# qfall/tools

Measured on AMD Instinct MI355X. Metric: preimages/sec (whole node) + HBM-BW% for samp_p, n=512 q~2^30 batch=4096, higher is better.
Workload: dtype f64+int64

## Files before the change

### tools_amd/csrc/psf_np_kernels.hpp

```cpp
#pragma once
#include <type_traits>
#include "psf_kernels.hpp"

namespace psf {

constexpr int NP_NB = 64;

__host__ __device__ inline size_t np_panel_rowblocks(size_t J) { return (J * NP_NB + 127) / 128; }
__host__ __device__ inline size_t np_panel_base(size_t J) { return 4 * ((J * J) / 4); }

__global__ __launch_bounds__(256) void k_np_gram(const int32_t* __restrict__ St, const double* __restrict__ Gt, size_t d, double* __restrict__ Gd) {
  __shared__ double sB[16][65];
  __shared__ double sG[16][65];
  const size_t j0 = (size_t)blockIdx.y * 64, i0 = (size_t)blockIdx.x * 64;
  const int tid = threadIdx.x, tx = tid & 15, ty = tid >> 4;
  if (i0 > j0 + 63) {
    for (int e = tid; e < 64 * 64; e += 256) {
      const size_t j = j0 + (e >> 6), i = i0 + (e & 63);
      if (j < d && i < d) Gd[j * d + i] = 0.0;
    }
    return;
  }
  double acc[4][4];
#pragma unroll
  for (int a = 0; a < 4; ++a)
#pragma unroll
    for (int b = 0; b < 4; ++b) acc[a][b] = 0.0;
  for (size_t t0 = 0; t0 < d; t0 += 16) {
    for (int e = tid; e < 64 * 16; e += 256) {
      const int r = e >> 4, tt = e & 15;
      const size_t t = t0 + tt;
      sB[tt][r] = (j0 + r < d && t < d) ? (double)St[(j0 + r) * d + t] : 0.0;
      sG[tt][r] = (i0 + r < d && t < d) ? Gt[(i0 + r) * d + t] : 0.0;
    }
    __syncthreads();
#pragma unroll
    for (int tt = 0; tt < 16; ++tt) {
      double bv[4], gv[4];
#pragma unroll
      for (int a = 0; a < 4; ++a) { bv[a] = sB[tt][ty * 4 + a]; gv[a] = sG[tt][tx * 4 + a]; }
#pragma unroll
      for (int a = 0; a < 4; ++a)
#pragma unroll
        for (int b = 0; b < 4; ++b) acc[a][b] = fma(bv[a], gv[b], acc[a][b]);
    }
    __syncthreads();
  }
#pragma unroll
  for (int a = 0; a < 4; ++a)
#pragma unroll
    for (int b = 0; b < 4; ++b) {
      const size_t j = j0 + ty * 4 + a, i = i0 + tx * 4 + b;
      if (j < d && i < d) Gd[j * d + i] = j > i ? acc[a][b] : 0.0;
    }
}

__global__ void k_np_pack_panels(const double* __restrict__ Gd, size_t d, size_t nblk, double* __restrict__ Gp) {
  const size_t total = np_panel_base(nblk) * TR_CHUNK;
  for (size_t g = (size_t)blockIdx.x * blockDim.x + threadIdx.x; g < total; g += (size_t)gridDim.x * blockDim.x) {
    const size_t chunk = g / TR_CHUNK;
    const int pos = (int)(g % TR_CHUNK);
    size_t J = (size_t)(2.0 * sqrt((double)(chunk / 4)));
    while (np_panel_base(J + 1) <= chunk) ++J;
    while (np_panel_base(J) > chunk) --J;
    const size_t rel = chunk - np_panel_base(J), rb = rel / 4, kc = rel % 4;
    const int ks = pos >> 9, tile = (pos >> 6) & 7, ln = pos & 63;
    const size_t i = rb * 128 + tile * 16 + (ln & 15);
    const size_t j = J * NP_NB + kc * 16 + ks * 4 + (ln >> 4);
    Gp[g] = (i < J * NP_NB && j < d) ? Gd[j * d + i] : 0.0;
  }
}
constexpr int NP_TRI = 2048;
__global__ void k_np_pack_inblock(const double* __restrict__ Gd, size_t d, size_t nblk, double* __restrict__ Gin) {
  const size_t total = nblk * NP_TRI;
  for (size_t g = (size_t)blockIdx.x * blockDim.x + threadIdx.x; g < total; g += (size_t)gridDim.x * blockDim.x) {
    const size_t J = g / NP_TRI, e = g % NP_TRI;
    double v = 0.0;
    if (e < (size_t)NP_NB * (NP_NB - 1) / 2) {
      size_t l = (size_t)((1.0 + sqrt(1.0 + 8.0 * (double)e)) * 0.5);
      while (l * (l - 1) / 2 > e) --l;
      while ((l + 1) * l / 2 <= e) ++l;
      const size_t li = e - l * (l - 1) / 2;
      const size_t j = J * NP_NB + l, i = J * NP_NB + li;
      if (j < d) v = Gd[j * d + i];
    }
// ... 740 lines not shown
  const int wr = wave >> 1, wc = wave & 1;
  const size_t row0 = (size_t)bi * TR_BM + wr * 32, col0 = (size_t)bj * TR_BN + wc * 64;
  d4 acc[2][4];
#pragma unroll
  for (int i = 0; i < 2; ++i)
#pragma unroll
    for (int j = 0; j < 4; ++j)
#pragma unroll
      for (int r = 0; r < 4; ++r) acc[i][j][r] = T[(row0 + i * 16 + (lane >> 4) + 4 * r) * ldt + col0 + j * 16 + (lane & 15)];
  const int nk = 4 * job.nsub;
  auto stage_load = [&](int kc, int buf) {
    const size_t Jb = (size_t)(job.J_first - (kc >> 2));
    const double* ga = Gp + (np_panel_base(Jb) + (size_t)bi * 4 + (size_t)(kc & 3)) * TR_CHUNK + lane * 2;
    const double* gb = Zf + ((size_t)bj * nkb + Jb * (NP_NB / 16) + (size_t)(kc & 3)) * TR_CHUNK + lane * 2;
    double* la = smem + buf * (2 * TR_CHUNK);
#pragma unroll
    for (int i = 0; i < 2; ++i) {
      const int piece = wave * 2 + i;
      __builtin_amdgcn_global_load_lds(ga + piece * 128, (lds_void_ptr)(la + piece * 128), 16, 0, 0);
      __builtin_amdgcn_global_load_lds(gb + piece * 128, (lds_void_ptr)(la + TR_CHUNK + piece * 128), 16, 0, COH ? 16 : 0);
    }
  };
  stage_load(0, 0);
  asm volatile("s_waitcnt vmcnt(0)" ::: "memory");
  __syncthreads();
  for (int kc = 0; kc < nk; ++kc) {
    const int cur = kc & 1;
    if (kc + 1 < nk) stage_load(kc + 1, cur ^ 1);
    const double* sA = smem + cur * (2 * TR_CHUNK);
    const double* sB = sA + TR_CHUNK;
#pragma unroll
    for (int ks = 0; ks < TR_BK / 4; ++ks) {
      double av[2], bv[4];
#pragma unroll
      for (int i = 0; i < 2; ++i) av[i] = -sA[(ks * 8 + wr * 2 + i) * 64 + lane];
#pragma unroll
      for (int i = 0; i < 4; ++i) bv[i] = sB[(ks * 8 + wc * 4 + i) * 64 + lane];
#pragma unroll
      for (int i = 0; i < 2; ++i)
#pragma unroll
        for (int j = 0; j < 4; ++j) acc[i][j] = __builtin_amdgcn_mfma_f64_16x16x4f64(av[i], bv[j], acc[i][j], 0, 0, 0);
    }
    asm volatile("s_waitcnt vmcnt(0)" ::: "memory");
    __syncthreads();
  }
#pragma unroll
  for (int i = 0; i < 2; ++i)
#pragma unroll
    for (int j = 0; j < 4; ++j)
#pragma unroll
      for (int r = 0; r < 4; ++r) {
        const size_t row = row0 + i * 16 + (lane >> 4) + 4 * r;
        if (row >= job.row_lo && row < job.row_hi) {
          if (COH) __hip_atomic_store(T + row * ldt + col0 + j * 16 + (lane & 15), acc[i][j][r], __ATOMIC_RELAXED, __HIP_MEMORY_SCOPE_AGENT);
          else T[row * ldt + col0 + j * 16 + (lane & 15)] = acc[i][j][r];
        }
      }
}

struct NpStepJobs { NpUpdateJob job[3]; unsigned ntiles[3]; };

template <int G>
__global__ __launch_bounds__(512, 4) void k_np_step(NpSampleArgs a, size_t dim, size_t J, uint64_t seed, uint32_t tag, uint64_t first_index, size_t B, unsigned nS,
                                                    NpStepJobs jobs, int nbj, const double* __restrict__ Gp, double* __restrict__ Tm) {
  extern __shared__ __attribute__((aligned(16))) unsigned char np_smem[];
  unsigned id = blockIdx.x;
  if (id < nS) { np_sample_body<G>(np_smem, id, a, dim, J, seed, tag, first_index, B); return; }
  id -= nS;
#pragma unroll
  for (int q = 0; q < 3; ++q) {
    if (id < jobs.ntiles[q]) { np_update_tile(reinterpret_cast<double*>(np_smem), id, jobs.job[q], nbj, Gp, a.Zf, a.nkb, Tm, a.ldt); return; }
    id -= jobs.ntiles[q];
  }
}

constexpr int NP_GW = 64;
constexpr int NP_WALK_SLOTS = 3;
struct NpWalkSync {
  unsigned* zcount;
  unsigned* tready;
  unsigned* abort;
  unsigned nblk_stride;
  unsigned spin_limit;
};

__device__ __forceinline__ bool np_walk_wait(const unsigned* word, unsigned target, unsigned* abort_word, unsigned spin_limit, int* s_flag) {
  if (threadIdx.x == 0) {
    int ok = 1;
    unsigned spins = 0;
    while (__hip_atomic_load(word, __ATOMIC_RELAXED, __HIP_MEMORY_SCOPE_AGENT) < target) {
      __builtin_amdgcn_s_sleep(2);
      if ((++spins & 255u) == 0 && __hip_atomic_load(abort_word, __ATOMIC_RELAXED, __HIP_MEMORY_SCOPE_AGENT) != 0) { ok = 0; break; }
      if (spins >= spin_limit) { __hip_atomic_store(abort_word, 1u, __ATOMIC_RELAXED, __HIP_MEMORY_SCOPE_AGENT); ok = 0; break; }
    }
    *s_flag = ok;
  }
  __syncthreads();
  const int ok = *s_flag;
  __syncthreads();
  return ok != 0;
}

template <int G>
__device__ __forceinline__ void np_walk_sampler(unsigned char* smem, unsigned wg, const NpSampleArgs& a, size_t dim, size_t nblk, uint64_t seed, uint32_t tag,
                                                uint64_t first_index, size_t B, const NpWalkSync& sy) {
  int* s_flag = reinterpret_cast<int*>(smem + 65536 - 16);
  const unsigned grp = wg / (unsigned)(NP_GW / (4 * G));
  long long zr[G];
#pragma unroll
  for (int s = 0; s < G; ++s) zr[s] = 0;
  for (size_t J = nblk; J-- > 0;) {
    if (J + 2 < nblk) {
      if (!np_walk_wait(sy.tready + (size_t)grp * sy.nblk_stride + J, 1u, sy.abort, sy.spin_limit, s_flag)) return;
    }
    np_sample_body<G, true, true>(smem, wg, a, dim, J, seed, tag, first_index, B, zr);
    asm volatile("s_waitcnt vmcnt(0)" ::: "memory");
    __syncthreads();
    if (threadIdx.x == 0 && J >= 2) __hip_atomic_fetch_add(sy.zcount + (size_t)grp * sy.nblk_stride + J, 1u, __ATOMIC_RELAXED, __HIP_MEMORY_SCOPE_AGENT);
  }
}

__device__ __forceinline__ void np_walk_updater(unsigned char* smem, unsigned grp, unsigned ul, unsigned ug, unsigned need, const NpSampleArgs& a, size_t nblk,
                                                const double* __restrict__ Gp, double* __restrict__ T, const NpWalkSync& sy) {
  double* s_z = reinterpret_cast<double*>(smem);
  int* s_flag = reinterpret_cast<int*>(smem + 65536 - 16);
  int* s_arr = reinterpret_cast<int*>(smem + 65536 - 32);
  const int tid = threadIdx.x, lane = tid & 63;
  const int wave = __builtin_amdgcn_readfirstlane(tid >> 6);
  const size_t col0 = (size_t)grp * NP_GW;
  const size_t ldt = a.ldt;
  const uint32_t t_lane = (uint32_t)(((size_t)(lane >> 4) * ldt + (size_t)(lane & 15)) * sizeof(double));
  const uint32_t f_lane = (uint32_t)(lane * sizeof(double));
  auto t_at = [&](size_t row, size_t col) -> double* {
    return reinterpret_cast<double*>(reinterpret_cast<char*>(T + row * ldt + col) + t_lane);
  };
  d4 acc[NP_WALK_SLOTS][4];
  long blk[NP_WALK_SLOTS];
#pragma unroll
  for (int sl = 0; sl < NP_WALK_SLOTS; ++sl) {
    const long k = 2 * sl + (wave >> 2);
    const long Jb = (long)ul + k * (long)ug;
    blk[sl] = Jb + 2 < (long)nblk ? Jb : -1;
    const size_t row0 = (size_t)(blk[sl] < 0 ? 0 : blk[sl]) * NP_NB + (size_t)(wave & 3) * 16;
#pragma unroll
    for (int nf = 0; nf < 4; ++nf)
#pragma unroll
      for (int r = 0; r < 4; ++r) acc[sl][nf][r] = blk[sl] < 0 ? 0.0 : *t_at(row0 + 4 * r, col0 + nf * 16);
  }
  if (tid == 0) *s_arr = 0;
  const size_t bj = col0 / TR_BN;
  const int t0 = (int)((col0 % TR_BN) / 16);
  for (size_t J = nblk; J-- > 2;) {
    if (!np_walk_wait(sy.zcount + (size_t)grp * sy.nblk_stride + J, need, sy.abort, sy.spin_limit, s_flag)) return;
    {
      const double* zsrc = a.Zf + (bj * a.nkb + J * (NP_NB / 16)) * TR_CHUNK;
#pragma unroll
      for (int i = 0; i < 8; ++i) {
        const int e = i * 8 + wave;
        const int kstep = e >> 2, nf = e & 3, kc = kstep >> 2, ks = kstep & 3;
        const double* src = reinterpret_cast<const double*>(reinterpret_cast<const char*>(zsrc + (size_t)kc * TR_CHUNK + (size_t)((ks * 8 + t0 + nf) * 64)) + f_lane);
        s_z[e * 64 + lane] = __hip_atomic_load(src, __ATOMIC_RELAXED, __HIP_MEMORY_SCOPE_AGENT);
      }
    }
    __syncthreads();
    const long Ju = (long)J - 2;
#pragma unroll
    for (int pass = 0; pass < 2; ++pass) {
#pragma unroll
      for (int sl = 0; sl < NP_WALK_SLOTS; ++sl) {
        const bool urgent = blk[sl] == Ju;
        if (blk[sl] < 0 || blk[sl] > Ju || urgent != (pass == 0)) continue;
        const size_t i0 = (size_t)blk[sl] * NP_NB + (size_t)(wave & 3) * 16;
        const double* ga = Gp + (np_panel_base(J) + (i0 / 128) * 4) * TR_CHUNK + ((i0 % 128) / 16) * 64;
#pragma unroll
        for (int kstep = 0; kstep < 16; ++kstep) {
          const double av = -*reinterpret_cast<const double*>(reinterpret_cast<const char*>(ga + (size_t)(kstep >> 2) * TR_CHUNK + (kstep & 3) * 512) + f_lane);
#pragma unroll
          for (int nf = 0; nf < 4; ++nf) acc[sl][nf] = __builtin_amdgcn_mfma_f64_16x16x4f64(av, s_z[(kstep * 4 + nf) * 64 + lane], acc[sl][nf], 0, 0, 0);
        }
        if (urgent) {
#pragma unroll
          for (int nf = 0; nf < 4; ++nf)
#pragma unroll
            for (int r = 0; r < 4; ++r)
              __hip_atomic_store(t_at((size_t)Ju * NP_NB + (size_t)(wave & 3) * 16 + 4 * r, col0 + nf * 16), acc[sl][nf][r], __ATOMIC_RELAXED, __HIP_MEMORY_SCOPE_AGENT);
          asm volatile("s_waitcnt vmcnt(0)" ::: "memory");
          if (lane == 0) {
            const int prev = __hip_atomic_fetch_add(s_arr, 1, __ATOMIC_RELAXED, __HIP_MEMORY_SCOPE_WORKGROUP);
            if ((prev & 3) == 3) __hip_atomic_store(sy.tready + (size_t)grp * sy.nblk_stride + (size_t)Ju, 1u, __ATOMIC_RELAXED, __HIP_MEMORY_SCOPE_AGENT);
          }
        }
      }
    }
    __syncthreads();
  }
}

template <int G>
__global__ __launch_bounds__(512, 4) void k_np_walk(NpSampleArgs a, size_t dim, size_t nblk, uint64_t seed, uint32_t tag, uint64_t first_index, size_t B, unsigned nS,
                                                    unsigned ngroups, unsigned ug, const double* __restrict__ Gp, double* __restrict__ Tm, NpWalkSync sy) {
  extern __shared__ __attribute__((aligned(16))) unsigned char np_smem[];
  unsigned id = blockIdx.x;
  if (id < nS) {
    np_walk_sampler<G>(np_smem, id, a, dim, nblk, seed, tag, first_index, B, sy);
  } else {
    id -= nS;
    const unsigned grp = id / ug, ul = id % ug;
    if (grp >= ngroups) return;
    const unsigned per = (unsigned)(NP_GW / (4 * G));
    const unsigned first = grp * per, need = nS - first < per ? nS - first : per;
    np_walk_updater(np_smem, grp, ul, ug, need, a, nblk, Gp, Tm, sy);
  }
}

template <int G>
__global__ __launch_bounds__(512, 4) void k_np_walk_solo(NpSampleArgs a, size_t dim, size_t nblk, uint64_t seed, uint32_t tag, uint64_t first_index, size_t B, const double* __restrict__ Gp,
                                                         double* __restrict__ Tm, const unsigned* __restrict__ only_if, unsigned long long* __restrict__ reruns) {
  extern __shared__ __attribute__((aligned(16))) unsigned char np_smem[];
  if (__hip_atomic_load(only_if, __ATOMIC_RELAXED, __HIP_MEMORY_SCOPE_AGENT) == 0) return;
  const unsigned wg = blockIdx.x;
  const int tid = threadIdx.x, lane = tid & 63;
  const int wave = __builtin_amdgcn_readfirstlane(tid >> 6);
  if (wg == 0 && tid == 0) atomicAdd(reruns, 1ull);
  long long zr[G];
#pragma unroll
  for (int s = 0; s < G; ++s) zr[s] = 0;
  const size_t b = (size_t)wg * 4 * G + (size_t)wave;
  const bool owner = wave < 4 * G && b < B;
  for (size_t J = nblk; J-- > 0;) {
    if (J + 2 < nblk) {
      __builtin_amdgcn_fence(__ATOMIC_ACQUIRE, "agent");
      if (owner) {
        const size_t i = J * NP_NB + (size_t)lane;
        double t = Tm[i * a.ldt + b];
        const double* zb = a.Zf + (b / TR_BN) * a.nkb * TR_CHUNK;
        const int bc = (int)(b % TR_BN);
        for (size_t Jb = nblk; Jb-- > J + 2;) {
          const double* gp = Gp + (np_panel_base(Jb) + (i / 128) * 4) * TR_CHUNK;
          const double* zp = zb + Jb * (NP_NB / 16) * TR_CHUNK;
#pragma unroll 4
          for (int kc = 0; kc < NP_NB / 16; ++kc)
#pragma unroll
            for (int kk = 0; kk < 16; ++kk)
              t = fma(-zp[(size_t)kc * TR_CHUNK + tr_chunk_pos(bc, kk)], gp[(size_t)kc * TR_CHUNK + tr_chunk_pos((int)(i % 128), kk)], t);
        }
        __hip_atomic_store(Tm + i * a.ldt + b, t, __ATOMIC_RELAXED, __HIP_MEMORY_SCOPE_AGENT);
      }
      asm volatile("s_waitcnt vmcnt(0)" ::: "memory");
      __syncthreads();
    }
    np_sample_body<G, true, true>(np_smem, wg, a, dim, J, seed, tag, first_index, B, zr);
    asm volatile("s_waitcnt vmcnt(0)" ::: "memory");
    __syncthreads();
  }
}

#ifdef PSF_EXPERIMENTS
template <int G>
struct NpWalk2Jobs {
  const double* Gp; double* T; const double* Zf;
  const unsigned* zcount_g; unsigned* tready_g; unsigned* abort_w; int* s_arr;
  size_t ldt, nkb, col0, bj;
  unsigned need, spin_limit;
  int nblk, t0, hw, HW, lane;
  uint32_t t_lane, f_lane;
  int Jn, fi, zmin;
  bool aborted;

  __device__ __forceinline__ bool spin(const unsigned* word, unsigned target) {
    unsigned spins = 0;
    while (__hip_atomic_load(word, __ATOMIC_RELAXED, __HIP_MEMORY_SCOPE_AGENT) < target) {
      if (aborted) return false;
      __builtin_amdgcn_s_sleep(2);
      if ((++spins & 255u) == 0 && __hip_atomic_load(abort_w, __ATOMIC_RELAXED, __HIP_MEMORY_SCOPE_AGENT) != 0) { aborted = true; return false; }
      if (spins >= spin_limit) { __hip_atomic_store(abort_w, 1u, __ATOMIC_RELAXED, __HIP_MEMORY_SCOPE_AGENT); aborted = true; return false; }
    }
    return true;
  }
  __device__ __forceinline__ bool wait_word(const unsigned* w) { return spin(w, 1u); }
  __device__ __forceinline__ int imax(int J) const {
    const int fmax = 4 * (J - 2) + 3;
    return fmax >= hw ? (fmax - hw) / HW : -1;
  }
  __device__ __forceinline__ double* t_at(size_t row, size_t col) const {
    return reinterpret_cast<double*>(reinterpret_cast<char*>(T + row * ldt + col) + t_lane);
// ... 356 lines not shown
```

### tools_amd/csrc/psfgpv_impl.hpp

```cpp

#include <algorithm>
#include "psf_hip_util.hpp"
struct NpBatch {
  size_t bcap = 0;
  DevArr<double> dTm;
  DevArr<double> dZf;
  DevArr<int8_t> dZ8;
  DevArr<double> dC0p;
  DevArr<uint64_t> dSol;
  DevArr<double> dC1;
  DevArr<int64_t> dE1;
  DevArr<unsigned> dWalk;
  DevArr<unsigned char> dZocc;
};
struct NpLane : NpBatch {
  size_t ld = 0, zplane = 0, walk_words = 0;
  DevArr<int> dFlags;
  int* dFail = nullptr;
};

struct psfgpv_handle {
  psfp_handle* base = nullptr;
  double s = 0;
  size_t n = 0, m = 0, dim = 0;
  DevArr<int32_t> dSt;
  DevArr<double> dGt;
  DevArr<double> dNorm2;
  DevArr<SampleZParams> dSz;
  DevArr<uint64_t> dT;
  DevArr<uint32_t> dPiv;
  size_t nblk = 0, dpad = 0, nrb = 0, nkc = 0, nkb = 0;
  DevArr<double> dGp;
  DevArr<double> dGin;
  DevArr<double> dGnx;
  DevArr<NpRow> dRows;
  DevArr<double> dBpiv;
  DevArr<int8_t> dB8;
  bool basis_hi = false, basis_generic = false;
  DevArr<unsigned char> dBocc;
  int np_combine = 1;
  NpLane ln[2];
  int last_lanes = 1;
  bool two_pass = false;
  size_t nkd = 0;
  DevArr<double> dBfull;
  int np_walk = -1;
  int cus = 0;
  int walk_slots[3] = {0, 0, 0};
  unsigned walk_spins = 1u << 22;
  int last_form = 0, last_G = 0;
  int last_parts = 1;
  int split_delay_us = 0;
  int np_split = 0;
  Stream sh[2];
  Event evFork, evHalf[2];
  int np_g = 0;
  int np_immediate = -1;
  bool has_key = false;
  bool timing = false;
  bool last_generic = false;
  Event ev[3];
  hipStream_t last_stream = nullptr;
};

static psf_status gpv_finish_basis(psfgpv_handle* g, bool compute_gso) {
  const size_t d = g->dim;
  KeygenClock kc("psfgpv");
  if (compute_gso) {
    hipLaunchKernelGGL(k_i32_to_f64, dim3(grid_for(d * d)), dim3(256), 0, 0, g->dSt, g->dGt, d * d);
    DevBuf dinfo;
    HIP_TRY(dinfo.alloc(sizeof(int)));
    HIP_TRY(dinfo.zero(sizeof(int)));
    if (gso_blocked(nullptr, g->dGt, d, d, dinfo.as<int>()) != hipSuccess) return PSF_ERR_HIP;
    int info = 0;
    dinfo.download(&info, sizeof(int));
    if (info != 0) return PSF_ERR_PARAM;
    kc.mark("  gso_blocked");
  }
  hipLaunchKernelGGL(k_row_norm2_chain, dim3((unsigned)((d + 63) / 64)), dim3(64), 0, 0, g->dGt, d, g->dNorm2);
  HIP_TRY(hipGetLastError());
  std::vector<double> norm2(d);
  HIP_TRY(hipMemcpy(norm2.data(), g->dNorm2, d * sizeof(double), hipMemcpyDeviceToHost));
  std::vector<SampleZParams> sz(d);
  for (size_t i = 0; i < d; ++i) {
    if (!(norm2[i] > 0.0)) return PSF_ERR_PARAM;
    sz[i] = make_sample_z_params(g->s / std::sqrt(norm2[i]));
  }
  HIP_TRY(hipMemcpy(g->dSz, sz.data(), d * sizeof(SampleZParams), hipMemcpyHostToDevice));
  {
    std::vector<NpRow> rows(g->nblk * NP_NB, NpRow{0.0, 0.f, 0, 1, 0, 0, 16});
    for (size_t i = 0; i < d; ++i) {
      const SampleZParams& p = sz[i];
      const bool fast = p.n_int < (1u << 24) && p.c6 < (1ll << 24);
      rows[i] = NpRow{1.0 / norm2[i], (float)(p.inv_s * 2.1289340388624525), fast ? (int32_t)p.c6 : 0, p.n_int, p.thr_int, p.thr_frac, fast ? p.sh : 0u};
    }
    HIP_TRY(hipMemcpy(g->dRows, rows.data(), rows.size() * sizeof(NpRow), hipMemcpyHostToDevice));
  }
  kc.mark("  norms, SampleZ rows");
  {
    DevBuf gram;
    HIP_TRY(gram.alloc(d * d * sizeof(double)));
    double* dGd = gram.as<double>();
    const unsigned tiles = (unsigned)((d + 63) / 64);
    hipLaunchKernelGGL(k_np_gram, dim3(tiles, tiles), dim3(256), 0, 0, g->dSt, g->dGt, d, dGd);
    if (np_panel_base(g->nblk))
      hipLaunchKernelGGL(k_np_pack_panels, dim3(grid_for(np_panel_base(g->nblk) * TR_CHUNK, 256, 256 * 64)), dim3(256), 0, 0, dGd, d, g->nblk, g->dGp);
    hipLaunchKernelGGL(k_np_pack_inblock, dim3(grid_for(g->nblk * NP_TRI)), dim3(256), 0, 0, dGd, d, g->nblk, g->dGin);
    hipLaunchKernelGGL(k_np_pack_next, dim3(grid_for(g->nblk * NP_NB * NP_NB)), dim3(256), 0, 0, dGd, d, g->nblk, g->dGnx);
    HIP_TRY(hipGetLastError());
    HIP_TRY(hipDeviceSynchronize());
  }
  kc.mark("  gram + packing");
  {
    DevBuf dinfo;
    HIP_TRY(dinfo.alloc(2 * sizeof(int)));
    HIP_TRY(dinfo.zero(2 * sizeof(int)));
    hipLaunchKernelGGL(k_np_pack_basis8, dim3(grid_for(g->dpad * g->dpad, 256, 256 * 64)), dim3(256), 0, 0, g->dSt, d, g->dpad, g->dB8, dinfo.as<int>());
    int info[2] = {0, 0};
    HIP_TRY(dinfo.download(info, sizeof(info)));
    g->basis_generic = info[0] != 0;
    g->basis_hi = info[1] != 0;
    hipLaunchKernelGGL(k_np_occ_basis, dim3((unsigned)(g->nrb * g->nrb), 2), dim3(256), 0, 0, g->dB8, g->dpad, (int)g->nrb, g->dBocc);
    HIP_TRY(hipGetLastError());
  }
  return PSF_OK;
}

static psf_status gpv_build_solver(psfgpv_handle* g) {
  psfp_handle* b = g->base;
  std::vector<uint64_t> A(b->n * b->m);
  HIP_TRY(hipMemcpy(A.data(), b->dA, A.size() * sizeof(uint64_t), hipMemcpyDeviceToHost));
  std::vector<uint32_t> piv;
  std::vector<uint64_t> T;
  const psf_status rc = solve_precompute(A.data(), b->n, b->m, b->q, piv, T);
  if (rc != PSF_OK) return rc;
  {
    const size_t nn = b->n;
    std::vector<size_t> order(nn);
    for (size_t r = 0; r < nn; ++r) order[r] = r;
    std::sort(order.begin(), order.end(), [&](size_t x, size_t y) { return piv[x] < piv[y]; });
    std::vector<uint32_t> piv2(nn);
    std::vector<uint64_t> T2(T.size());
    for (size_t r = 0; r < nn; ++r) {
      piv2[r] = piv[order[r]];
      for (size_t t = 0; t < nn; ++t) T2[r * nn + t] = T[order[r] * nn + t];
    }
    piv.swap(piv2);
    T.swap(T2);
  }
  {
    const size_t nn = b->n;
    std::vector<uint64_t> Tt(T.size());
    for (size_t r = 0; r < nn; ++r)
      for (size_t t = 0; t < nn; ++t) Tt[t * nn + r] = T[r * nn + t];
    HIP_TRY(hipMemcpy(g->dT, Tt.data(), Tt.size() * sizeof(uint64_t), hipMemcpyHostToDevice));
  }
  HIP_TRY(hipMemcpy(g->dPiv, piv.data(), piv.size() * sizeof(uint32_t), hipMemcpyHostToDevice));
  hipLaunchKernelGGL(k_np_pack_bpiv, dim3(grid_for(g->nrb * g->nkc * TR_CHUNK, 256, 256 * 64)), dim3(256), 0, 0, g->dGt, g->dPiv, g->dim, g->n, g->nrb, g->nkc, g->dBpiv);
  if (g->two_pass)
    hipLaunchKernelGGL(k_np_pack_bpiv, dim3(grid_for(g->nrb * g->nkd * TR_CHUNK, 256, 256 * 64)), dim3(256), 0, 0, g->dGt, (const uint32_t*)nullptr, g->dim, g->dim, g->nrb, g->nkd, g->dBfull);
  HIP_TRY(hipGetLastError());
  HIP_TRY(hipDeviceSynchronize());
  return PSF_OK;
}

static psf_status ensure_np_batch(psfgpv_handle* g, NpLane& L, size_t B) {
  if (B <= L.bcap) return PSF_OK;
  HIP_TRY(hipDeviceSynchronize());
  static_cast<NpBatch&>(L) = NpBatch{};
  const size_t ld = round_up(B, TR_BN);
  L.ld = ld;
  HIP_TRY(L.dTm.alloc(g->dpad * ld));
  HIP_TRY(L.dZf.alloc(ld * g->nkb * 16));
  L.zplane = g->dpad * ld;
  HIP_TRY(L.dZ8.alloc(3 * L.zplane));
  HIP_TRY(L.dZocc.alloc(2 * (ld / 128) * g->nrb));
  HIP_TRY(L.dC0p.alloc(ld * g->nkc * 16));
  HIP_TRY(L.dSol.alloc(g->n * ld));
  if (g->two_pass) {
    HIP_TRY(L.dC1.alloc(ld * g->nkd * 16));
    HIP_TRY(L.dE1.alloc(B * g->dim));
  }
  L.walk_words = round_up(2 * (ld / NP_GW) * g->nblk + 4, 4);
  HIP_TRY(L.dWalk.alloc(L.walk_words));
  HIP_TRY(hipMemset(L.dTm, 0, g->dpad * ld * sizeof(double)));
  HIP_TRY(hipMemset(L.dZf, 0, ld * g->nkb * 16 * sizeof(double)));
  HIP_TRY(hipMemset(L.dZ8, 0, 3 * L.zplane));
  HIP_TRY(hipDeviceSynchronize());
  L.bcap = B;
  return PSF_OK;
}

static psf_status launch_np_recombination(psfgpv_handle* g, NpLane& L, hipStream_t st, size_t B, int64_t* d_e, int pass, size_t col0 = 0);

struct WalkTurn {
  static constexpr int MAX_DEV = 64;
  static std::mutex& mu() { static std::mutex m; return m; }
  static hipEvent_t* events() { static hipEvent_t ev[MAX_DEV] = {}; return ev; }
  static bool* recorded() { static bool r[MAX_DEV] = {}; return r; }
  std::unique_lock<std::mutex> lk;
  int dev; hipStream_t st;
  WalkTurn(int device, hipStream_t s) : lk(mu()), dev(device), st(s) {
    if (dev < 0 || dev >= MAX_DEV) { dev = -1; return; }
    if (!events()[dev] && hipEventCreateWithFlags(&events()[dev], hipEventDisableTiming) != hipSuccess) { events()[dev] = nullptr; dev = -1; return; }
    if (recorded()[dev]) hipStreamWaitEvent(st, events()[dev], 0);
  }
  ~WalkTurn() {
    if (dev >= 0 && hipEventRecord(events()[dev], st) == hipSuccess) recorded()[dev] = true;
  }
};

struct NpCols {
  double* Tm; double* Zf; int8_t* Z8; unsigned char* Zocc; double* C0p; double* C1; uint64_t* Sol; int64_t* E1;
};
static NpCols np_cols(const psfgpv_handle* g, const NpLane& L, size_t col0) {
  const size_t cb = col0 / TR_BN;
  return NpCols{L.dTm + col0, L.dZf + cb * g->nkb * TR_CHUNK, L.dZ8 + col0 * 16, L.dZocc + cb * g->nrb, L.dC0p + cb * g->nkc * TR_CHUNK,
                L.dC1 ? L.dC1 + cb * g->nkd * TR_CHUNK : nullptr, L.dSol + col0, L.dE1 ? L.dE1 + col0 * g->dim : nullptr};
}

static bool np_walk_fits(const psfgpv_handle* g, size_t B, int* Gw_out, unsigned* nSw_out, unsigned* ngroups_out, unsigned* ug_out) {
  if (g->np_walk == 0 || g->np_walk == 3 || g->cus <= 0 || g->nblk < 3) return false;
  if (!psf_experiments_build && g->np_g != 1 && B > 4 * (size_t)g->cus) return false;
  const int Gw = (g->np_g == 1 || g->np_g == 2) ? g->np_g : (B <= 4 * (size_t)g->cus ? 1 : 2);
  const unsigned nSw = (unsigned)((B + 4 * (size_t)Gw - 1) / (4 * (size_t)Gw));
  const unsigned per = (unsigned)(NP_GW / (4 * Gw)), ngroups = (nSw + per - 1) / per;
  const long slots = (long)g->cus * (long)g->walk_slots[Gw];
  unsigned ug = 0;
  if (ngroups && nSw <= (unsigned)g->cus && slots > (long)nSw) ug = (unsigned)std::min<long>((slots - (long)nSw) / (long)ngroups, (long)g->cus / (long)ngroups);
  if (ug > g->nblk - 2) ug = (unsigned)(g->nblk - 2);
  if (!(nSw <= (unsigned)g->cus && ug >= 1 && (size_t)2 * NP_WALK_SLOTS * ug >= g->nblk - 2)) return false;
  if (Gw_out) { *Gw_out = Gw; *nSw_out = nSw; *ngroups_out = ngroups; *ug_out = ug; }
  return true;
}

static psf_status launch_nearest_plane(psfgpv_handle* g, NpLane& L, hipStream_t st, uint64_t seed, uint32_t tag, uint64_t first_index, size_t B, int64_t* d_e, int pass = 0, size_t col0 = 0,
                                       bool may_walk = true) {
  const size_t ld = L.ld, nbj = round_up(B, TR_BN) / TR_BN;
  const size_t lds_gemm = 4 * TR_CHUNK * sizeof(double);
  const NpCols v = np_cols(g, L, col0);
  int* const flags = L.dFlags + 4 * pass;
  if (pass == 0) hipLaunchKernelGGL(k_np_project, dim3((unsigned)nbj, (unsigned)g->nrb), dim3(256), lds_gemm, st, g->dBpiv, g->nkc, v.C0p, g->nkc, (int)g->nkc, v.Tm, ld);
  else hipLaunchKernelGGL(k_np_project, dim3((unsigned)nbj, (unsigned)g->nrb), dim3(256), lds_gemm, st, g->dBfull, g->nkd, v.C1, g->nkd, (int)g->nkd, v.Tm, ld);
  int G = g->np_g;
  if (G != 1 && G != 2) G = B <= 2048 ? 1 : 2;
  NpSampleArgs a{v.Tm, ld, g->dGin, g->dGnx, g->dRows, g->dSz, v.Zf, g->nkb, v.Z8, L.zplane, ld, flags};
  {
    int Gw = 0; unsigned nSw = 0, ngroups = 0, ug = 0;
    if (may_walk && col0 == 0 && np_walk_fits(g, B, &Gw, &nSw, &ngroups, &ug)) {
      NpWalkSync sy{L.dWalk, L.dWalk + (size_t)ngroups * g->nblk, L.dWalk + (size_t)2 * ngroups * g->nblk, (unsigned)g->nblk, g->walk_spins};
      NpSampleArgs aw{L.dTm, ld, g->dGin, g->dGnx, g->dRows, g->dSz, L.dZf, g->nkb, L.dZ8, L.zplane, ld, flags};
      const unsigned ntot = nSw + ngroups * ug;
      unsigned long long* reruns = reinterpret_cast<unsigned long long*>(L.dFlags + 8);
      {
        WalkTurn turn(g->base->prm.device, st);
        hipMemsetAsync(L.dWalk, 0, L.walk_words * sizeof(unsigned), st);
        if (Gw == 1) hipLaunchKernelGGL((k_np_walk<1>), dim3(ntot), dim3(512), 65536, st, aw, g->dim, g->nblk, seed, tag, first_index, B, nSw, ngroups, ug, g->dGp, L.dTm, sy);
#ifdef PSF_EXPERIMENTS
        else hipLaunchKernelGGL((k_np_walk<2>), dim3(ntot), dim3(512), 65536, st, aw, g->dim, g->nblk, seed, tag, first_index, B, nSw, ngroups, ug, g->dGp, L.dTm, sy);
#endif
      }
      if (pass == 0) hipLaunchKernelGGL(k_np_project, dim3((unsigned)nbj, (unsigned)g->nrb), dim3(256), lds_gemm, st, g->dBpiv, g->nkc, L.dC0p, g->nkc, (int)g->nkc, L.dTm, ld, (const unsigned*)sy.abort);
      else hipLaunchKernelGGL(k_np_project, dim3((unsigned)nbj, (unsigned)g->nrb), dim3(256), lds_gemm, st, g->dBfull, g->nkd, L.dC1, g->nkd, (int)g->nkd, L.dTm, ld, (const unsigned*)sy.abort);
      if (Gw == 1) hipLaunchKernelGGL((k_np_walk_solo<1>), dim3(nSw), dim3(512), 65536, st, aw, g->dim, g->nblk, seed, tag, first_index, B, g->dGp, L.dTm, (const unsigned*)sy.abort, reruns);
#ifdef PSF_EXPERIMENTS
      else hipLaunchKernelGGL((k_np_walk_solo<2>), dim3(nSw), dim3(512), 65536, st, aw, g->dim, g->nblk, seed, tag, first_index, B, g->dGp, L.dTm, (const unsigned*)sy.abort, reruns);
#endif
      g->last_form = 1; g->last_G = Gw;
      return launch_np_recombination(g, L, st, B, d_e, pass, col0);
    }
  }
  const unsigned nS = (unsigned)((B + 4 * (size_t)G - 1) / (4 * (size_t)G));
#ifdef PSF_EXPERIMENTS
  if (g->np_walk == 3 && col0 == 0 && g->cus > 0 && g->nblk >= 3 && nS <= 2u * (unsigned)g->cus) {
    const unsigned per = (unsigned)(NP_GW / (4 * G)), ngroups = (nS + per - 1) / per;
    NpWalkSync sy{L.dWalk, L.dWalk + (size_t)ngroups * g->nblk, L.dWalk + (size_t)2 * ngroups * g->nblk, (unsigned)g->nblk, g->walk_spins};
    hipMemsetAsync(L.dWalk, 0, L.walk_words * sizeof(unsigned), st);
    if (G == 1) hipLaunchKernelGGL((k_np_walk2<1>), dim3(nS), dim3(512), 65536, st, a, g->dim, g->nblk, seed, tag, first_index, B, nS, g->dGp, L.dTm, sy);
    else hipLaunchKernelGGL((k_np_walk2<2>), dim3(nS), dim3(512), 65536, st, a, g->dim, g->nblk, seed, tag, first_index, B, nS, g->dGp, L.dTm, sy);
    g->last_form = 3; g->last_G = G;
    return launch_np_recombination(g, L, st, B, d_e, pass, col0);
  }
#endif
  const size_t W = NP_PANEL;
  const bool immediate = g->np_immediate >= 0 ? g->np_immediate != 0 : B <= 2048;
  for (size_t J = g->nblk; J-- > 0;) {
    NpStepJobs jobs;
    for (int q = 0; q < 3; ++q) { jobs.job[q] = NpUpdateJob{0, 0, 0, 0, 0, 0}; jobs.ntiles[q] = 0; }
    auto set_job = [&](int q, size_t J_first, size_t nsub, size_t rb0, size_t rb1, size_t lo, size_t hi) {
      if (rb1 <= rb0 || hi <= lo) return;
      jobs.job[q] = NpUpdateJob{(int)J_first, (int)nsub, (int)rb0, (int)(rb1 - rb0), lo, hi};
      jobs.ntiles[q] = (unsigned)((rb1 - rb0) * nbj);
    };
    if (J + 1 < g->nblk) {
      const size_t P = (J + 1) / W;
      const size_t lo = (P >= 1 && !immediate) ? (P - 1) * W * NP_NB : 0, hi = J * NP_NB;
      set_job(0, J + 1, 1, lo / 128, (hi + 127) / 128, lo, hi);
    }
    const size_t Pj = J / W, P = Pj + 1;
    if (P * W < g->nblk && P >= 2 && !immediate) {
      const size_t top = std::min(g->nblk, (P + 1) * W) - 1, nsub = top - P * W + 1;
      const size_t near_lo = (P - 2) * W * NP_NB, near_hi = (P - 1) * W * NP_NB;
      const size_t i = (P * W - 1) - J;
      if (i == 0) set_job(1, top, nsub, near_lo / 128, near_hi / 128, near_lo, near_hi);
      if (i == 0) set_job(2, top, nsub, 0, near_lo / 128, 0, near_lo);
    }
    const unsigned ntot = nS + jobs.ntiles[0] + jobs.ntiles[1] + jobs.ntiles[2];
    if (G == 1) hipLaunchKernelGGL((k_np_step<1>), dim3(ntot), dim3(512), 65536, st, a, g->dim, J, seed, tag, first_index, B, nS, jobs, (int)nbj, g->dGp, v.Tm);
    else hipLaunchKernelGGL((k_np_step<2>), dim3(ntot), dim3(512), 65536, st, a, g->dim, J, seed, tag, first_index, B, nS, jobs, (int)nbj, g->dGp, v.Tm);
  }
  g->last_form = 0; g->last_G = G;
  return launch_np_recombination(g, L, st, B, d_e, pass, col0);
}

static psf_status launch_np_recombination(psfgpv_handle* g, NpLane& L, hipStream_t st, size_t B, int64_t* d_e, int pass, size_t col0) {
  const size_t ld = L.ld;
  const NpCols v = np_cols(g, L, col0);
  int* const flags = L.dFlags + 4 * pass;
  const psfp_handle* b = g->base;
  const dim3 cgrid((unsigned)((B + 127) / 128), (unsigned)(g->dpad / 128));
  const int nk128 = (int)(g->dpad / 128);
  if (!g->basis_generic && g->np_combine != 0) {
    hipLaunchKernelGGL(k_np_occ_z, dim3((unsigned)(cgrid.x * g->nrb), 2), dim3(256), 0, st, v.Z8, L.zplane, ld, nk128, v.Zocc);
    hipLaunchKernelGGL(k_np_combine8_fused, cgrid, dim3(256), 65536 + 768, st, g->dB8, g->dpad, g->dim, nk128, g->basis_hi ? 2 : 1, g->dBocc, v.Z8, L.zplane, ld, B, v.Zocc, d_e, g->dim);
    if (pass == 0) hipLaunchKernelGGL(k_np_add_sol, dim3(grid_for(g->n * B)), dim3(256), 0, st, v.Sol, g->dPiv, g->n, B, ld, d_e, g->dim);
  }
#ifdef PSF_EXPERIMENTS
  else if (!g->basis_generic) {
    const size_t plane = g->dpad * g->dpad;
    const int8_t* zp[3] = {v.Z8, v.Z8 + L.zplane, v.Z8 + 2 * L.zplane};
    const int* gate[3] = {nullptr, flags + 1, flags + 2};
    bool first = true;
    for (int zi = 0; zi < 3; ++zi)
// ... 27 lines not shown
extern "C" void psf_debug_np_single(unsigned long long* out, int reset) {
  if (out) hipMemcpyFromSymbol(out, HIP_SYMBOL(g_np_single), sizeof(unsigned long long) * 8);
  if (reset) { unsigned long long z[8] = {0}; hipMemcpyToSymbol(HIP_SYMBOL(g_np_single), z, sizeof(z)); }
}
#endif
extern "C" void psf_debug_np_events(unsigned long long* out, int reset) {
  if (out) hipMemcpyFromSymbol(out, HIP_SYMBOL(g_np_events), sizeof(unsigned long long) * 4);
  if (reset) { unsigned long long z[4] = {0}; hipMemcpyToSymbol(HIP_SYMBOL(g_np_events), z, sizeof(z)); }
}
#endif

extern "C" {

static psf_status psfgpv_init(psfgpv_handle* g);

psf_status psfgpv_create(const psfgpv_params* prm, psfgpv_handle** out) {
  if (!prm || !out || !(prm->s > 0.0)) return PSF_ERR_PARAM;
  psfp_params bp;
  bp.gp = prm->gp; bp.r = 1.0; bp.s = prm->s; bp.device = prm->device; bp.flags = PSFP_FLAG_NO_PERTURB;
  psfp_handle* b = nullptr;
  const psf_status rc = psfp_create(&bp, &b);
  if (rc != PSF_OK) return rc;
  psfgpv_handle* g = new psfgpv_handle();
  g->base = b; g->s = prm->s; g->n = b->n; g->m = b->m; g->dim = b->m;
  const psf_status rc2 = psfgpv_init(g);
  if (rc2 != PSF_OK) { psfgpv_destroy(g); return rc2; }
  *out = g;
  return PSF_OK;
}

static psf_status psfgpv_init(psfgpv_handle* g) {
  const size_t d = g->dim;
  g->nblk = (d + NP_NB - 1) / NP_NB;
  g->dpad = round_up(d, 128);
  g->nrb = g->dpad / 128;
  g->nkc = round_up(g->n, 16) / 16;
  g->nkb = round_up(d, NP_NB) / 16;
  HIP_TRY(g->dSt.alloc(d * d));
  HIP_TRY(g->dGt.alloc(d * d));
  HIP_TRY(g->dNorm2.alloc(d));
  HIP_TRY(g->dSz.alloc(d));
  HIP_TRY(g->dT.alloc(g->n * g->n));
  HIP_TRY(g->dPiv.alloc(g->n));
  HIP_TRY(g->dGp.alloc((np_panel_base(g->nblk) + 1) * TR_CHUNK));
  HIP_TRY(g->dGin.alloc(g->nblk * NP_TRI));
  HIP_TRY(g->dGnx.alloc(g->nblk * NP_NB * NP_NB));
  HIP_TRY(g->dRows.alloc(g->nblk * NP_NB));
  HIP_TRY(g->dBpiv.alloc(g->nrb * g->nkc * TR_CHUNK));
  HIP_TRY(g->dB8.alloc(2 * g->dpad * g->dpad));
  HIP_TRY(g->dBocc.alloc(2 * g->nrb * g->nrb));
  HIP_TRY(g->ln[0].dFlags.alloc(12));
  HIP_TRY(hipMemset(g->ln[0].dFlags, 0, 12 * sizeof(int)));
  g->ln[0].dFail = g->base->dFail;
  g->two_pass = (double)g->base->q * std::sqrt((double)g->n) > g->s * 8192.0;
  { const char* ev = psf_exp_env("PSF_NP_TWO_PASS"); if (ev) g->two_pass = atoi(ev) != 0; }
  g->nkd = round_up(d, 16) / 16;
  if (g->two_pass) HIP_TRY(g->dBfull.alloc(g->nrb * g->nkd * TR_CHUNK));
  { const char* ev = psf_exp_env("PSF_NP_G"); g->np_g = ev ? atoi(ev) : 0; }
  { const char* ev = psf_exp_env("PSF_NP_IMMEDIATE"); g->np_immediate = ev ? (atoi(ev) != 0 ? 1 : 0) : -1; }
  HIP_TRY(hipFuncSetAttribute(reinterpret_cast<const void*>(k_np_project), hipFuncAttributeMaxDynamicSharedMemorySize, 4 * TR_CHUNK * sizeof(double)));
  HIP_TRY(hipFuncSetAttribute(reinterpret_cast<const void*>(k_np_step<1>), hipFuncAttributeMaxDynamicSharedMemorySize, 65536));
  HIP_TRY(hipFuncSetAttribute(reinterpret_cast<const void*>(k_np_step<2>), hipFuncAttributeMaxDynamicSharedMemorySize, 65536));
  HIP_TRY(hipFuncSetAttribute(reinterpret_cast<const void*>(k_np_walk<1>), hipFuncAttributeMaxDynamicSharedMemorySize, 65536));
#ifdef PSF_EXPERIMENTS
  HIP_TRY(hipFuncSetAttribute(reinterpret_cast<const void*>(k_np_walk<2>), hipFuncAttributeMaxDynamicSharedMemorySize, 65536));
#endif
#ifdef PSF_EXPERIMENTS
  HIP_TRY(hipFuncSetAttribute(reinterpret_cast<const void*>(k_np_walk2<1>), hipFuncAttributeMaxDynamicSharedMemorySize, 65536));
  HIP_TRY(hipFuncSetAttribute(reinterpret_cast<const void*>(k_np_walk2<2>), hipFuncAttributeMaxDynamicSharedMemorySize, 65536));
  HIP_TRY(hipFuncSetAttribute(reinterpret_cast<const void*>(k_np_combine8<false>), hipFuncAttributeMaxDynamicSharedMemorySize, 65536));
  HIP_TRY(hipFuncSetAttribute(reinterpret_cast<const void*>(k_np_combine8<true>), hipFuncAttributeMaxDynamicSharedMemorySize, 65536));
#endif
  { int cu = 0; HIP_TRY(hipDeviceGetAttribute(&cu, hipDeviceAttributeMultiprocessorCount, g->base->prm.device)); g->cus = cu; }
  HIP_TRY(hipFuncSetAttribute(reinterpret_cast<const void*>(k_np_walk_solo<1>), hipFuncAttributeMaxDynamicSharedMemorySize, 65536));
#ifdef PSF_EXPERIMENTS
  HIP_TRY(hipFuncSetAttribute(reinterpret_cast<const void*>(k_np_walk_solo<2>), hipFuncAttributeMaxDynamicSharedMemorySize, 65536));
#endif
  HIP_TRY(hipOccupancyMaxActiveBlocksPerMultiprocessor(&g->walk_slots[1], reinterpret_cast<const void*>(k_np_walk<1>), 512, 65536));
#ifdef PSF_EXPERIMENTS
  HIP_TRY(hipOccupancyMaxActiveBlocksPerMultiprocessor(&g->walk_slots[2], reinterpret_cast<const void*>(k_np_walk<2>), 512, 65536));
#endif
  if (const char* e = psf_exp_env("PSF_NP_WALK")) g->np_walk = std::atoi(e);
  if (const char* e = psf_exp_env("PSF_NP_WALK_SPINS")) { const long v = std::atol(e); if (v >= 1) g->walk_spins = (unsigned)v; }
  HIP_TRY(hipFuncSetAttribute(reinterpret_cast<const void*>(k_np_combine8_fused), hipFuncAttributeMaxDynamicSharedMemorySize, 65536 + 768));
  if (const char* e = psf_exp_env("PSF_NP_COMBINE")) g->np_combine = std::atoi(e);
  for (auto& e : g->ev) HIP_TRY(hipEventCreate(e.put()));
#ifdef PSF_EXPERIMENTS
  for (auto& sx : g->sh) HIP_TRY(hipStreamCreateWithFlags(sx.put(), hipStreamNonBlocking));
  HIP_TRY(hipEventCreateWithFlags(g->evFork.put(), hipEventDisableTiming));
  for (auto& e : g->evHalf) HIP_TRY(hipEventCreateWithFlags(e.put(), hipEventDisableTiming));
#endif
  if (const char* e = psf_exp_env("PSF_NP_SPLIT")) { const int v = std::atoi(e); if (v >= 0 && v <= 2) g->np_split = v; }
  if (const char* e = psf_exp_env("PSF_NP_SPLIT_DELAY")) { const int v = std::atoi(e); if (v >= 0 && v <= 1000) g->split_delay_us = v; }
  return PSF_OK;
}

void psfgpv_destroy(psfgpv_handle* g) {
  if (!g) return;
  psfp_handle* const base = g->base;
  hipSetDevice(base->prm.device);
  base->hp.quiesce();
  delete g;
  psfp_destroy(base);
}

size_t psfgpv_m(const psfgpv_handle* g) { return g ? g->m : 0; }

psf_status psfgpv_trap_gen(psfgpv_handle* g, uint64_t seed) {
  if (!g) return PSF_ERR_PARAM;
  psfp_handle* b = g->base;
  HIP_TRY(hipSetDevice(b->prm.device));
  PSFP_QUIESCE(b);
  g->has_key = false;
  KeygenClock kc("psfgpv");
  psf_status rc = gen_A_R(b, seed);
  if (rc != PSF_OK) return rc;
  kc.mark("A, R");
  DevBuf bt;
  const size_t ldw = b->ldr;
  HIP_TRY(bt.alloc(b->m * ldw));
  int8_t* dBT = bt.as<int8_t>();
  const int reversed = is_power_of_base(b->prm.gp.base, b->k, b->q) ? 1 : 0;
  hipLaunchKernelGGL(k_gpv_bottom_t, dim3(grid_for(b->m * ldw, 256, 256 * 64)), dim3(256), 0, 0, b->dA, b->m, (uint32_t)b->n, (uint32_t)b->k, b->mb, b->w,
                     b->q, b->prm.gp.base, b->dSk, reversed, dBT, ldw);
  hipLaunchKernelGGL(k_gpv_basis_t, dim3((unsigned)((b->mb + 63) / 64), (unsigned)((b->m + 63) / 64)), dim3(256), 0, 0, dBT, ldw, b->dR, b->ldr, b->m,
                     b->mb, b->w, g->dSt);
  hipLaunchKernelGGL(k_gpv_basis_t_tail, dim3(grid_for(b->m * b->w, 256, 256 * 64)), dim3(256), 0, 0, dBT, ldw, b->m, b->mb, b->w, g->dSt);
  HIP_TRY(hipGetLastError());
  HIP_TRY(hipDeviceSynchronize());
  kc.mark("short basis");
  rc = gpv_finish_basis(g, true);
  if (rc != PSF_OK) return rc;
  kc.mark("gso + walk operands");
  rc = gpv_build_solver(g);
  if (rc != PSF_OK) return rc;
  kc.mark("solve operator");
  b->has_key = true; b->has_pub = true;
  g->has_key = true;
  return PSF_OK;
}

psf_status psfgpv_load_key(psfgpv_handle* g, const uint64_t* A, const int32_t* basis_t, const double* gso_t) {
  if (!g || !A || !basis_t || !gso_t) return PSF_ERR_PARAM;
  psfp_handle* b = g->base;
  HIP_TRY(hipSetDevice(b->prm.device));
  PSFP_QUIESCE(b);
  g->has_key = false;
  HIP_TRY(hipMemcpy(b->dA, A, b->n * b->m * sizeof(uint64_t), hipMemcpyHostToDevice));
  split_A(b);
  HIP_TRY(hipMemcpy(g->dSt, basis_t, g->dim * g->dim * sizeof(int32_t), hipMemcpyHostToDevice));
  HIP_TRY(hipMemcpy(g->dGt, gso_t, g->dim * g->dim * sizeof(double), hipMemcpyHostToDevice));
  psf_status rc = gpv_finish_basis(g, false);
  if (rc != PSF_OK) return rc;
  rc = gpv_build_solver(g);
  if (rc != PSF_OK) return rc;
  b->has_key = true; b->has_pub = true;
  g->has_key = true;
  return PSF_OK;
}

psf_status psfgpv_export_key(const psfgpv_handle* g, uint64_t* A, int8_t* R, int32_t* basis_t, double* gso_t) {
  if (!g) return PSF_ERR_PARAM;
  if (!g->has_key) return PSF_ERR_NO_KEY;
  const psfp_handle* b = g->base;
  HIP_TRY(hipSetDevice(b->prm.device));
  if (A) HIP_TRY(hipMemcpy(A, b->dA, b->n * b->m * sizeof(uint64_t), hipMemcpyDeviceToHost));
// ... 591 lines not shown
```

Measured before the change: 70070.

## Assign walk kernel sampler/updater roles dynamically by XCD and CU via atomic tickets

```diff
diff --git a/tools_amd/csrc/psf_np_kernels.hpp b/tools_amd/csrc/psf_np_kernels.hpp
--- a/tools_amd/csrc/psf_np_kernels.hpp
+++ b/tools_amd/csrc/psf_np_kernels.hpp
@@ -1,6 +1,7 @@
 #pragma once
 #include <type_traits>
 #include "psf_kernels.hpp"
+#include "psf_np_roles.hpp"
 
 namespace psf {
 
@@ -907,6 +908,10 @@
   unsigned* abort;
   unsigned nblk_stride;
   unsigned spin_limit;
+  unsigned* tickets;
+  unsigned role_cus;
+  unsigned nxcd;
+  unsigned role_grain;
 };
 
 __device__ __forceinline__ bool np_walk_wait(const unsigned* word, unsigned target, unsigned* abort_word, unsigned spin_limit, int* s_flag) {
@@ -1021,11 +1026,32 @@
   }
 }
 
+__device__ __forceinline__ unsigned np_walk_task(unsigned char* smem, unsigned nS, unsigned ngroups, unsigned ug, unsigned per, const NpWalkSync& sy) {
+  if (sy.role_cus == 0) return blockIdx.x;
+  unsigned* s_task = reinterpret_cast<unsigned*>(smem + 65536 - 48);
+  if (threadIdx.x == 0) {
+    unsigned xcc, hwid;
+    asm volatile("s_getreg_b32 %0, hwreg(HW_REG_XCC_ID)" : "=s"(xcc));
+    asm volatile("s_getreg_b32 %0, hwreg(HW_REG_HW_ID)" : "=s"(hwid));
+    const NpRoleGrid g{nS, ngroups, ug, per, sy.nxcd};
+    unsigned* tickets = sy.tickets;
+    NpRoleTask task{NP_ROLE_SAMPLER, 0u};
+    const bool got = np_role_take(g, (xcc & 15u) % sy.nxcd, np_role_of_cu((hwid >> 8) & 15u, sy.role_cus, sy.role_grain),
+                                  [tickets](unsigned list) { return __hip_atomic_fetch_add(tickets + list, 1u, __ATOMIC_RELAXED, __HIP_MEMORY_SCOPE_AGENT); }, &task);
+    *s_task = !got ? ~0u : task.role == NP_ROLE_SAMPLER ? task.id : nS + task.id;
+  }
+  __syncthreads();
+  const unsigned id = __builtin_amdgcn_readfirstlane(*s_task);
+  __syncthreads();
+  return id;
+}
+
 template <int G>
 __global__ __launch_bounds__(512, 4) void k_np_walk(NpSampleArgs a, size_t dim, size_t nblk, uint64_t seed, uint32_t tag, uint64_t first_index, size_t B, unsigned nS,
                                                     unsigned ngroups, unsigned ug, const double* __restrict__ Gp, double* __restrict__ Tm, NpWalkSync sy) {
   extern __shared__ __attribute__((aligned(16))) unsigned char np_smem[];
-  unsigned id = blockIdx.x;
+  unsigned id = np_walk_task(np_smem, nS, ngroups, ug, (unsigned)(NP_GW / (4 * G)), sy);
+  if (id == ~0u) return;
   if (id < nS) {
     np_walk_sampler<G>(np_smem, id, a, dim, nblk, seed, tag, first_index, B, sy);
   } else {
diff --git a/tools_amd/csrc/psf_np_roles.hpp b/tools_amd/csrc/psf_np_roles.hpp
--- /dev/null
+++ b/tools_amd/csrc/psf_np_roles.hpp
@@ -0,0 +1,54 @@
+#pragma once
+
+#if defined(__HIPCC__) || defined(__CUDACC__)
+#define PSF_NP_HD __host__ __device__
+#else
+#define PSF_NP_HD
+#endif
+
+namespace psf {
+
+constexpr unsigned NP_ROLE_MAX_XCDS = 8;
+enum : int { NP_ROLE_SAMPLER = 0, NP_ROLE_UPDATER = 1 };
+
+struct NpRoleGrid { unsigned nS, ngroups, ug, per, nxcd; };
+struct NpRoleList { unsigned xcd; int role; };
+struct NpRoleTask { int role; unsigned id; };
+
+PSF_NP_HD inline int np_role_of_cu(unsigned cu_id, unsigned role_cus, unsigned grain = 1) {
+  return (cu_id / grain) % role_cus == role_cus - 1 ? NP_ROLE_UPDATER : NP_ROLE_SAMPLER;
+}
+
+PSF_NP_HD inline unsigned np_role_groups(const NpRoleGrid& g, unsigned x) { return x < g.ngroups ? (g.ngroups - x + g.nxcd - 1) / g.nxcd : 0u; }
+
+PSF_NP_HD inline unsigned np_role_count(const NpRoleGrid& g, unsigned x, int role) {
+  const unsigned ng = np_role_groups(g, x);
+  if (ng == 0) return 0u;
+  if (role == NP_ROLE_UPDATER) return ng * g.ug;
+  const unsigned last = x + (ng - 1) * g.nxcd;
+  return (ng - 1) * g.per + (last == g.ngroups - 1 ? g.nS - last * g.per : g.per);
+}
+
+PSF_NP_HD inline NpRoleTask np_role_task(const NpRoleGrid& g, unsigned x, int role, unsigned t) {
+  const unsigned w = role == NP_ROLE_UPDATER ? g.ug : g.per;
+  const unsigned grp = x + (t / w) * g.nxcd;
+  return NpRoleTask{role, grp * w + t % w};
+}
+
+PSF_NP_HD inline NpRoleList np_role_list(const NpRoleGrid& g, unsigned x, int role, unsigned p) {
+  return NpRoleList{(x + p / 2) % g.nxcd, (p & 1u) ? 1 - role : role};
+}
+
+template <class FetchAdd>
+PSF_NP_HD inline bool np_role_take(const NpRoleGrid& g, unsigned x, int role, FetchAdd&& fetch_add, NpRoleTask* out) {
+  for (unsigned p = 0; p < 2 * g.nxcd; ++p) {
+    const NpRoleList l = np_role_list(g, x, role, p);
+    const unsigned cnt = np_role_count(g, l.xcd, l.role);
+    if (cnt == 0) continue;
+    const unsigned t = fetch_add(2 * l.xcd + (unsigned)l.role);
+    if (t < cnt) { *out = np_role_task(g, l.xcd, l.role, t); return true; }
+  }
+  return false;
+}
+
+}
diff --git a/tools_amd/csrc/psfgpv_impl.hpp b/tools_amd/csrc/psfgpv_impl.hpp
--- a/tools_amd/csrc/psfgpv_impl.hpp
+++ b/tools_amd/csrc/psfgpv_impl.hpp
@@ -48,6 +48,9 @@
   int cus = 0;
   int walk_slots[3] = {0, 0, 0};
   unsigned walk_spins = 1u << 22;
+  unsigned np_role_cus = 2;
+  unsigned np_role_grain = 1;
+  unsigned np_role_xcds = 0;
   int last_form = 0, last_G = 0;
   int last_parts = 1;
   int split_delay_us = 0;
@@ -181,7 +184,7 @@
     HIP_TRY(L.dC1.alloc(ld * g->nkd * 16));
     HIP_TRY(L.dE1.alloc(B * g->dim));
   }
-  L.walk_words = round_up(2 * (ld / NP_GW) * g->nblk + 4, 4);
+  L.walk_words = round_up(2 * (ld / NP_GW) * g->nblk + 4 + 2 * NP_ROLE_MAX_XCDS, 4);
   HIP_TRY(L.dWalk.alloc(L.walk_words));
   HIP_TRY(hipMemset(L.dTm, 0, g->dpad * ld * sizeof(double)));
   HIP_TRY(hipMemset(L.dZf, 0, ld * g->nkb * 16 * sizeof(double)));
@@ -248,7 +251,9 @@
   {
     int Gw = 0; unsigned nSw = 0, ngroups = 0, ug = 0;
     if (may_walk && col0 == 0 && np_walk_fits(g, B, &Gw, &nSw, &ngroups, &ug)) {
-      NpWalkSync sy{L.dWalk, L.dWalk + (size_t)ngroups * g->nblk, L.dWalk + (size_t)2 * ngroups * g->nblk, (unsigned)g->nblk, g->walk_spins};
+      const unsigned nxcd = g->np_role_xcds ? g->np_role_xcds : (g->cus >= 64 && g->cus % (int)NP_ROLE_MAX_XCDS == 0 ? NP_ROLE_MAX_XCDS : 1u);
+      unsigned* const abort_w = L.dWalk + (size_t)2 * ngroups * g->nblk;
+      NpWalkSync sy{L.dWalk, L.dWalk + (size_t)ngroups * g->nblk, abort_w, (unsigned)g->nblk, g->walk_spins, abort_w + 4, g->np_role_cus, nxcd, g->np_role_grain};
       NpSampleArgs aw{L.dTm, ld, g->dGin, g->dGnx, g->dRows, g->dSz, L.dZf, g->nkb, L.dZ8, L.zplane, ld, flags};
       const unsigned ntot = nSw + ngroups * ug;
       unsigned long long* reruns = reinterpret_cast<unsigned long long*>(L.dFlags + 8);
@@ -442,6 +447,9 @@
 #endif
   if (const char* e = psf_exp_env("PSF_NP_WALK")) g->np_walk = std::atoi(e);
   if (const char* e = psf_exp_env("PSF_NP_WALK_SPINS")) { const long v = std::atol(e); if (v >= 1) g->walk_spins = (unsigned)v; }
+  if (const char* e = psf_exp_env("PSF_NP_ROLE_CUS")) { const int v = std::atoi(e); if (v == 0 || (v >= 2 && v <= 16)) g->np_role_cus = (unsigned)v; }
+  if (const char* e = psf_exp_env("PSF_NP_ROLE_GRAIN")) { const int v = std::atoi(e); if (v >= 1 && v <= 16) g->np_role_grain = (unsigned)v; }
+  if (const char* e = psf_exp_env("PSF_NP_ROLE_XCDS")) { const int v = std::atoi(e); if (v >= 1 && v <= (int)NP_ROLE_MAX_XCDS) g->np_role_xcds = (unsigned)v; }
   HIP_TRY(hipFuncSetAttribute(reinterpret_cast<const void*>(k_np_combine8_fused), hipFuncAttributeMaxDynamicSharedMemorySize, 65536 + 768));
   if (const char* e = psf_exp_env("PSF_NP_COMBINE")) g->np_combine = std::atoi(e);
   for (auto& e : g->ev) HIP_TRY(hipEventCreate(e.put()));
```

Measured after the change: 70110, median of 3. Within noise of the previous version (+0.1%).
